# Mattdl/CLsurvey

Measured on AMD Instinct MI355X. Metric: images/sec (train+importance pass), EWC small_VGG9 Tiny-ImageNet task batch, higher is better.
Workload: dtype f32 (bf16x6 split operands on the conv fwd/bwd-data matrix products, fp32 accumulate); 1 GPU; EWC small_VGG9_cl_128_128, Tiny-ImageNet shapes (3x64x64, 20 classes), batch 200: train step + Fisher step (BASELINE configs[1]); batch=200, parallelism=1 GPU

## Files before the change

clsurvey_amd/_lib.py:

```python
import ctypes as C
import os

_HERE = os.path.dirname(os.path.abspath(__file__))
LIB_PATH = os.path.join(_HERE, "libclhip.so")

_p = C.c_void_p
_i = C.c_int
_f = C.c_float
_z = C.c_size_t
_l = C.c_long


class HatParam(C.Structure):
    _fields_ = [("theta", _p), ("grad", _p), ("buf", _p), ("mask_back", _p), ("n", _z), ("is_emb", _i), ("reserved", _i)]


class HatGateJob(C.Structure):
    _fields_ = [("emb_row", _p), ("gate", _p), ("mask_pre", _p), ("n", _i), ("reserved", _i)]


class HatLayer(C.Structure):
    _fields_ = [("w", _p), ("gate_in", _p), ("out", _p), ("K", _z), ("C", _z), ("R", _z)]


# ... 92 lines not shown
    "clhip_axpy": (_i, [_p, _p, _z, _f, _i, _p]),
    "clhip_gem_gram_ws": (_z, [_i]),
    "clhip_gem_gram": (_i, [_p, _z, C.POINTER(_i), _i, _z, _p, _p, _z, _p]),
    "clhip_gem_project": (_i, [_p, _z, C.POINTER(_i), C.POINTER(_f), _i, _p, _p, _z, _p]),
    "clhip_gem_qp": (_i, [_p, _i, C.c_double, C.c_double, _p, _p, _p]),
    "clhip_gem_project_dev": (_i, [_p, _z, C.POINTER(_i), _p, _p, _i, _p, _p, _z, _p]),
    "clhip_net_create": (_i, [C.POINTER(LayerDesc), _i, _i, _i, _i, _i, C.POINTER(_p)]),
    "clhip_net_set_dropout": (_i, [_p, _i, _p, _l]),
    "clhip_net_set_bn": (_i, [_p, _i, _p, _p, _f, _f]),
    "clhip_net_set_training": (_i, [_p, _i]),
    "clhip_net_probe": (_i, [_p, _i]),
    "clhip_net_probe_read": (_i, [_p, C.POINTER(_f), C.POINTER(_i)]),
    "clhip_net_layer_input": (_i, [_p, _i, _p, _p]),
    "clhip_net_layer_pool_idx": (_i, [_p, _i, _p, _p]),
    "clhip_net_layer_paths": (_i, [_p, _i]),
    "clhip_net_probe_kind": (_i, [_p, _i, _i]),
    "clhip_net_set_input_grad": (_i, [_p, _i, _p]),
    "clhip_sigmoid_fwd": (_i, [_p, _p, _z, _p]),
    "clhip_sigmoid_bwd": (_i, [_p, _p, _p, _z, _p]),
    "clhip_mse_mean": (_i, [_p, _p, _z, _f, _p, _p, _p]),
    "clhip_adadelta_step": (_i, [_p, _p, _p, _p, _z, _f, _f, _f, _f, _p]),
    "clhip_bn_ws": (_z, [_i]),
    "clhip_bn_fwd": (_i, [_p, _p, _p, _p, _p, _p, _p, _p, _i, _i, _i, _i, _f, _f, _i, _p, _z, _p]),
    "clhip_bn_bwd": (_i, [_p, _p, _p, _p, _p, _p, _p, _p, _p, _i, _i, _i, _i, _i, _p, _z, _p]),
    "clhip_net_destroy": (None, [_p]),
    "clhip_net_workspace_bytes": (_z, [_p]),
    "clhip_net_num_classes": (_i, [_p]),
    "clhip_net_forward": (_i, [_p, _p, _p, _i, _p, _p, _p]),
    "clhip_net_backward": (_i, [_p, _p, _p, _p, _i, _p, _p, _p]),
    "clhip_net_loss_step": (_i, [_p, _p, _p, _p, _p, _i, _i, _p, _p, _p, _p, _p]),
# ... 40 lines not shown
```

clsurvey_amd/csrc/bswgrad.hip:

```cpp
#include "common.hpp"
#include <cstdlib>

namespace {

typedef __bf16 bw_bf16x8 __attribute__((ext_vector_type(8)));
typedef __bf16 bw_bf16x2 __attribute__((ext_vector_type(2)));
typedef float bw_f32x2 __attribute__((ext_vector_type(2)));


__device__ __forceinline__ unsigned bw_pk(float lo, float hi) {
    bw_f32x2 v = {lo, hi};
    return __builtin_bit_cast(unsigned, __builtin_convertvector(v, bw_bf16x2));
}
__device__ __forceinline__ void bw_split2(float a, float b, unsigned& p0, unsigned& p1, unsigned& p2) {
    p0 = bw_pk(a, b);
    float ra = a - __uint_as_float(p0 << 16), rb = b - __uint_as_float(p0 & 0xffff0000u);
    p1 = bw_pk(ra, rb);
    ra -= __uint_as_float(p1 << 16);
    rb -= __uint_as_float(p1 & 0xffff0000u);
    p2 = bw_pk(ra, rb);
}

struct BwA { clhip_u32x4 p[3]; };
struct BwB { unsigned p[3][5]; };

__device__ __forceinline__ bw_bf16x8 bw_op(unsigned a, unsigned b, unsigned c, unsigned d) {
    return __builtin_bit_cast(bw_bf16x8, clhip_u32x4{a, b, c, d});
}
template <int S>
__device__ __forceinline__ bw_bf16x8 bw_tap(const BwB& b, int i) {
    if constexpr (S == 0) return bw_op(b.p[i][0], b.p[i][1], b.p[i][2], b.p[i][3]);
    else if constexpr (S == 2) return bw_op(b.p[i][1], b.p[i][2], b.p[i][3], b.p[i][4]);
    else return bw_op(__builtin_amdgcn_alignbit(b.p[i][1], b.p[i][0], 16), __builtin_amdgcn_alignbit(b.p[i][2], b.p[i][1], 16),
                      __builtin_amdgcn_alignbit(b.p[i][3], b.p[i][2], 16), __builtin_amdgcn_alignbit(b.p[i][4], b.p[i][3], 16));
}

#if BW_ABL & 1
__device__ __forceinline__ floatx16 bw_fake_mfma(bw_bf16x8 a, bw_bf16x8 b, floatx16 c) {
    c[0] += __builtin_bit_cast(clhip_u32x4, a).x == 0x12345678u ? 1.f : 0.f;
    c[1] += __builtin_bit_cast(clhip_u32x4, b).y == 0x12345678u ? 1.f : 0.f;
    return c;
}
#define BW_MFMA(a, b, c) bw_fake_mfma(a, b, c)
#else
#define BW_MFMA(a, b, c) __builtin_amdgcn_mfma_f32_32x32x16_bf16(a, b, c, 0, 0, 0)
#endif

struct BwRawX { float4 lo, hi; float l, r; };
struct BwRawD { float4 lo, hi; unsigned codes; };

#ifndef BW_ABL
#define BW_ABL 0
#endif
#ifndef BW_SCHED
#define BW_SCHED 1
#endif

template <bool UNPOOL>
__global__ __launch_bounds__(256, 1) void bs_wgrad_kernel(const float* __restrict__ x, const float* __restrict__ dy,
                                                          const uint8_t* __restrict__ idx, float* __restrict__ part, int N, int C, int K,
                                                          int H, int W, int splits, long long rows_total, size_t slab_stride) {
    const int lane = threadIdx.x & 63, wave = threadIdx.x >> 6;
    const int col = lane & 31, half = lane >> 5;
    const int split = blockIdx.x % splits, bt = blockIdx.x / splits;
    const int c_tiles = C >> 6;
    const int ct = bt % c_tiles, kt = bt / c_tiles;
    const int k0 = kt * 64 + (wave & 1) * 32, c0 = ct * 64 + (wave >> 1) * 32;
    const int strips = W >> 4;
// ... 240 lines not shown
```

clsurvey_amd/csrc/common.hpp:

```cpp
#pragma once
#include <hip/hip_runtime.h>
#include <stdint.h>
#include <stddef.h>
#include "../../include/clhip.h"

#define CLHIP_LAUNCH_CHECK()                          \
    do {                                              \
        hipError_t e__ = hipGetLastError();           \
        if (e__ != hipSuccess) return (int)e__;       \
    } while (0)

static inline hipStream_t as_stream(void* s) { return reinterpret_cast<hipStream_t>(s); }

static inline bool aligned16(const void* p) { return (reinterpret_cast<uintptr_t>(p) & 15u) == 0; }

static inline int ew_grid(size_t work_items, int block) {
    size_t g = (work_items + block - 1) / block;
    if (g < 1) g = 1;
    if (g > 2048) g = 2048;
    return (int)g;
}

static __device__ __attribute__((aligned(16))) float clhip_zero16[4] = {0.f, 0.f, 0.f, 0.f};

// ... 71 lines not shown
int clhip_internal_fc_bwd_combo(const clhip_gemm_args* g, int gemm_blocks, const clhip_fc_chain* d, float* grads, const float* x,
                                int N, const float* acts, const float* dlogits, const float* dz, hipStream_t s);

int clhip_internal_fc_tail_ok(const clhip_fc_chain* d);
int clhip_internal_fc_tail(const clhip_fc_chain* d, const float* params, float* acts, int N, const int64_t* labels,
                           int reduction, int col_off, int ncols, float* dlogits, float* fcdz, float* loss_out, double* stats,
                           void* row_scratch, unsigned* counter, int do_loss, int do_bwd, const float* h1_slabs, int live,
                           hipStream_t s);
int clhip_internal_fc_fwd_partial(const float* x, const float* w, int M, int I, int O, void* ws, size_t ws_bytes, int* live,
                                  hipStream_t s);

#define CLHIP_WGRAD_JOBS_MAX 32
struct clhip_wgrad_job { const float* part; float* dw; float* db; int K, C, splits; int taps; };
int clhip_internal_conv3x3_wgrad_partial(const float* x, const float* dy, const uint8_t* unpool_idx, float* dw, float* db, int N,
                                         int C, int K, int H, int W, void* ws, size_t ws_bytes, void* stream, clhip_wgrad_job* job);
int clhip_internal_wgrad_reduce_multi(const clhip_wgrad_job* jobs, int n, hipStream_t s);

bool clhip_internal_convkk_ok(int N, int Cin, int Cout, int H, int W, int R, int S, int stride, int pad);
int clhip_internal_convkk(int mode, const float* in, const float* w, const float* bias, const float* mask_src, float* out, int N,
                          int Cin, int Cout, int H, int W, int relu, hipStream_t s);

struct clhip_wino_wt { const float* w; float* U; int Ko, Ci, mode, pad; };
int clhip_internal_wino_weights(const clhip_wino_wt* jobs, int n, hipStream_t s);
int clhip_internal_weight_images(const clhip_wino_wt* wino_jobs, int n_wino, const clhip_wino_wt* bs_jobs, int n_bs, hipStream_t s);
int clhip_internal_wino_conv_u(int mode, const float* in, const float* U, const float* bias, const float* mask_src, float* out,
                               uint8_t* pool_idx, int unpool, int N, int Cin, int Cout, int H, int W, int relu, hipStream_t s);
bool clhip_internal_wino_ok(int Cin, int Cout, int H, int W);
size_t clhip_internal_wino_ws(int Cin, int Cout);
bool clhip_internal_bs_ok(int Cin, int Cout, int H, int W);
bool clhip_internal_bs_preferred(int Cin, int Cout, int H, int W);
// ... 32 lines not shown
```

clsurvey_amd/csrc/conv3x3_wgrad.hip:

```cpp
#include <cstdlib>
#include "common.hpp"

namespace {

constexpr int KT = 64, CT = 64;

#ifdef CLHIP_TRACE
__device__ unsigned long long* g_wtrace = nullptr;
#define TR_NOW() __builtin_amdgcn_s_memtime()
#endif

template <int TW, int TH>
struct WGeo {
    static constexpr int BP = TW * TH;
    static constexpr int TWP = TW + 2;
    static constexpr int PLANE = (TH + 2) * TWP;
    static constexpr int PLANEP = PLANE | 1;
    static constexpr int LDP = BP + 1;
    static_assert(BP == 64, "stage is 64 pixels");
};

__device__ __forceinline__ void decode_stage(int st, int tiles_w, int tiles_h, int TW, int TH,
                                             int& n, int& h0, int& w0) {
    int tw_i = st % tiles_w;
// ... 519 lines not shown
    }
}

#ifndef CLHIP_U3
#define CLHIP_U3 1
#endif
#ifndef CLHIP_U3_BSUM_MFMA
#define CLHIP_U3_BSUM_MFMA 0
#endif
#ifndef CLHIP_U3_LDSDY
#define CLHIP_U3_LDSDY 1
#endif
constexpr int U3_DYROW = 20, U3_DY = 32 * U3_DYROW;
constexpr int U3_TWP = 35, U3_PLANE = 3 * U3_TWP, U3_HALO = 3 * U3_PLANE + 5;

__global__ __launch_bounds__(256) void conv3x3_wgrad_c3_unpool_kernel(
    const float* __restrict__ x, const float* __restrict__ dyp, float* __restrict__ part,
    int N, int C, int K, int H, int W, int tiles_w, int tiles_h, int total_stages, int splits, size_t slab_stride,
    const uint8_t* __restrict__ pool_idx) {
    __shared__ float halo[4 * 2 * U3_HALO];
    __shared__ float red[2 * 16 * 64 + 64];
#if CLHIP_U3_LDSDY
    __shared__ __attribute__((aligned(16))) float dyl[4 * 2 * U3_DY];
#endif
#if CLHIP_U3_BSUM_MFMA
    __shared__ float ones_s[64];
    ones_s[threadIdx.x & 63] = 1.f;
    __syncthreads();
#endif
    const int tid = threadIdx.x, lane = tid & 63, wave = tid >> 6;
    const int wk = wave & 1, wh = wave >> 1;
    const int li = lane & 31, kk = lane >> 5;
    const int split = blockIdx.x % splits;
    const int kt = blockIdx.x / splits;
    const int k0 = kt * KT;
    const int per = total_stages / splits, extra = total_stages % splits;
    const int st_begin = split * per + min(split, extra);
    const int st_end = st_begin + per + (split < extra ? 1 : 0);

    floatx16 acc;
#pragma unroll
    for (int r = 0; r < 16; ++r) acc[r] = 0.f;
    double bsum = 0.0;

    const int ncol = C * 9;
    int col_off = 0;
    if (li < ncol) {
        const int cc = li / 9, rs = li - cc * 9;
        col_off = cc * U3_PLANE + (rs / 3) * U3_TWP + (rs % 3);
// ... 138 lines not shown
                if (kr < K) slab[((size_t)rs * K + kr) * C + cc] = acc[r] + red[(wk * 16 + r) * 64 + lane];
            }
        }
#if CLHIP_U3_BSUM_MFMA
        if (li == ncol) {
#pragma unroll
            for (int r = 0; r < 16; ++r) {
                const int kr = k0 + wk * 32 + mfma32_row(r, lane);
                if (kr < K) slab[(size_t)9 * K * C + kr] = acc[r] + red[(wk * 16 + r) * 64 + lane];
            }
        }
#else
        if (kk == 0 && kok) slab[(size_t)9 * K * C + k] = (float)(bsum + (double)red[2048 + wk * 32 + li]);
#endif
    }
}

constexpr int RED_EL = 64, RED_J = 16, RED_V = 4;
constexpr int RED_THREADS = RED_EL / RED_V * RED_J;

template <int EL, int J>
__device__ __forceinline__ void wgrad_reduce_block(const float* __restrict__ part, float* __restrict__ dw, float* __restrict__ db,
                                                   int K, int C, int splits, size_t e0, double (*partial)[EL], int T = 9) {
    const size_t kc = (size_t)K * C, nw = (size_t)T * kc, total = nw + K;
    const int v = threadIdx.x % (EL / RED_V), j = threadIdx.x / (EL / RED_V);
    const size_t e = e0 + (size_t)v * RED_V;
    const int q = (splits + J - 1) / J;
    const int s0 = j * q, s1 = min(splits, s0 + q);
    double s[RED_V] = {0.0, 0.0, 0.0, 0.0};
    if ((total & 3) == 0 && e + RED_V <= total) {
#pragma unroll 4
        for (int sp = s0; sp < s1; ++sp) {
            const float4 t = *reinterpret_cast<const float4*>(part + (size_t)sp * total + e);
            s[0] += (double)t.x; s[1] += (double)t.y; s[2] += (double)t.z; s[3] += (double)t.w;
        }
    } else {
        for (int sp = s0; sp < s1; ++sp)
#pragma unroll
            for (int t = 0; t < RED_V; ++t)
                if (e + t < total) s[t] += (double)part[(size_t)sp * total + e + t];
    }
#pragma unroll
    for (int t = 0; t < RED_V; ++t) partial[j][v * RED_V + t] = s[t];
    __syncthreads();
    if (threadIdx.x < EL) {
        const int el = threadIdx.x;
        const size_t ee = e0 + el;
        if (ee < total) {
            double t = 0.0;
#pragma unroll
            for (int jj = 0; jj < J; ++jj) t += partial[jj][el];
            if (ee < nw) {
                const size_t rs = ee / kc, rem = ee - rs * kc;
                dw[rem * T + rs] = (float)t;
            } else if (db) {
                db[ee - nw] = (float)t;
            }
        }
    }
}

template <int EL, int J>
__global__ __launch_bounds__(RED_THREADS) void wgrad_reduce_kernel(const float* __restrict__ part, float* __restrict__ dw,
                                                                   float* __restrict__ db, int K, int C, int splits) {
    __shared__ double partial[J][EL];
    wgrad_reduce_block<EL, J>(part, dw, db, K, C, splits, (size_t)blockIdx.x * EL, partial);
}

struct RedJobs {
    clhip_wgrad_job job[CLHIP_WGRAD_JOBS_MAX];
    unsigned first[CLHIP_WGRAD_JOBS_MAX + 1];
    int n;
};

template <int EL, int JL>
__global__ __launch_bounds__(RED_THREADS) void wgrad_reduce_multi_kernel(RedJobs jobs) {
    __shared__ double partial[JL][EL];
    int ji = 0;
    while (ji + 1 < jobs.n && blockIdx.x >= jobs.first[ji + 1]) ++ji;
    const clhip_wgrad_job J = jobs.job[ji];
    wgrad_reduce_block<EL, JL>(J.part, J.dw, J.db, J.K, J.C, J.splits, (size_t)(blockIdx.x - jobs.first[ji]) * EL, partial, J.taps ? J.taps : 9);
}

struct WPlan {
    int TW, TH, tiles_w, tiles_h, total_stages, splits, k_tiles, c_tiles, group, groups, ps;
    size_t slab, ws_floats;
};

WPlan make_plan(int N, int C, int K, int H, int W) {
    WPlan p;
    if (W > 16) { p.TW = 32; p.TH = 2; }
    else if (W > 8) { p.TW = 16; p.TH = 4; }
    else { p.TW = 8; p.TH = 8; }
    p.tiles_w = (W + p.TW - 1) / p.TW;
    p.tiles_h = (H + p.TH - 1) / p.TH;
    p.total_stages = p.tiles_w * p.tiles_h * N;
    const bool smallc = (C * 9 <= 32);
// ... 37 lines not shown

#ifdef CLHIP_TRACE
int clhip_debug_set_wgrad_trace(void* p) {
    unsigned long long* q = static_cast<unsigned long long*>(p);
    return (int)hipMemcpyToSymbol(HIP_SYMBOL(g_wtrace), &q, sizeof(q));
}
#endif

size_t clhip_conv3x3_bwd_weight_ws(int N, int C, int K, int H, int W) {
    if (N <= 0 || C <= 0 || K <= 0 || H <= 0 || W <= 0) return 0;
    return make_plan(N, C, K, H, W).ws_floats * sizeof(float);
}

static int bwd_weight_impl(const float* x, const float* dy, const uint8_t* unpool_idx, float* dw, float* db,
                           int N, int C, int K, int H, int W, void* ws, size_t ws_bytes, void* stream,
                           clhip_wgrad_job* defer = nullptr) {
    if (!x || !dy || !dw || !ws || N <= 0 || C <= 0 || K <= 0 || H <= 0 || W <= 0) return CLHIP_EINVAL;
    if (unpool_idx && ((H & 1) || (W & 1))) return CLHIP_ENOTSUP;
    WPlan p = make_plan(N, C, K, H, W);
    if (ws_bytes < p.ws_floats * sizeof(float)) return CLHIP_ENOSPC;
    hipStream_t s = as_stream(stream);
    float* part = static_cast<float*>(ws);
    const bool smallc = (C * 9 <= 32);
    unsigned grid = (unsigned)(p.k_tiles * p.c_tiles * p.splits);
#define WG_ARGS x, dy, part, N, C, K, H, W, p.tiles_w, p.tiles_h, p.total_stages, p.splits
    if (CLHIP_U3 && smallc && unpool_idx && p.TW == 32 && W % 32 == 0 && aligned16(dy) && aligned16(unpool_idx) &&
        (size_t)N * K * H * W < ((size_t)1 << 31) && (size_t)N * C * H * W < ((size_t)1 << 29)) {
        hipLaunchKernelGGL(conv3x3_wgrad_c3_unpool_kernel, dim3(grid), dim3(256), 0, s, WG_ARGS, p.slab, unpool_idx);
    } else if (smallc) {
        if (p.TW == 32) hipLaunchKernelGGL((conv3x3_wgrad_smallc_kernel<32, 2>), dim3(grid), dim3(256), 0, s, WG_ARGS, p.slab, unpool_idx);
        else if (p.TW == 16) hipLaunchKernelGGL((conv3x3_wgrad_smallc_kernel<16, 4>), dim3(grid), dim3(256), 0, s, WG_ARGS, p.slab, unpool_idx);
        else hipLaunchKernelGGL((conv3x3_wgrad_smallc_kernel<8, 8>), dim3(grid), dim3(256), 0, s, WG_ARGS, p.slab, unpool_idx);
    } else {
        const bool vec = (W % 4 == 0) && (W % p.TW == 0) && aligned16(x) && aligned16(dy);
        if (unpool_idx && (!vec || (reinterpret_cast<uintptr_t>(unpool_idx) & 1u))) return CLHIP_ENOTSUP;
#define WG_K(TW_, TH_, VEC_, PS_, UNP_) hipLaunchKernelGGL((conv3x3_wgrad_kernel<TW_, TH_, VEC_, PS_, UNP_>), dim3(grid), dim3(256), 0, s, \
                                                           WG_ARGS, p.c_tiles, p.slab, unpool_idx)
#define WG_LAUNCH1(TW_, TH_, PS_) do { if (unpool_idx) WG_K(TW_, TH_, true, PS_, true); else if (vec) WG_K(TW_, TH_, true, PS_, false); \
                                      else WG_K(TW_, TH_, false, PS_, false); } while (0)
#define WG_LAUNCH(TW_, TH_) do { if (p.ps) WG_LAUNCH1(TW_, TH_, true); else WG_LAUNCH1(TW_, TH_, false); } while (0)
        if (p.TW == 32) WG_LAUNCH(32, 2);
        else if (p.TW == 16) WG_LAUNCH(16, 4);
        else WG_LAUNCH(8, 8);
// ... 39 lines not shown
    const unsigned bx = (unsigned)((slab + RED_EL - 1) / RED_EL);
    hipLaunchKernelGGL((wgrad_reduce_kernel<RED_EL, RED_J>), dim3(bx), dim3(RED_THREADS), 0, as_stream(stream),
                            static_cast<const float*>(ws), dw, db, K, C, splits);
    CLHIP_LAUNCH_CHECK();
    return 0;
}

}

int clhip_internal_conv3x3_wgrad_partial(const float* x, const float* dy, const uint8_t* unpool_idx, float* dw, float* db, int N,
                                         int C, int K, int H, int W, void* ws, size_t ws_bytes, void* stream, clhip_wgrad_job* job) {
    if (!job) return CLHIP_EINVAL;
    return bwd_weight_impl(x, dy, unpool_idx, dw, db, N, C, K, H, W, ws, ws_bytes, stream, job);
}

int clhip_internal_wgrad_reduce_multi(const clhip_wgrad_job* jobs, int n, hipStream_t s) {
    if (n <= 0) return 0;
    if (!jobs || n > CLHIP_WGRAD_JOBS_MAX) return CLHIP_EINVAL;
    RedJobs r;
    r.n = n;
    r.first[0] = 0;
    for (int i = 0; i < n; ++i) {
        r.job[i] = jobs[i];
        const size_t total = (size_t)(jobs[i].taps ? jobs[i].taps : 9) * jobs[i].K * jobs[i].C + jobs[i].K;
        r.first[i + 1] = r.first[i] + (unsigned)((total + RED_EL - 1) / RED_EL);
    }
    for (int i = n; i < CLHIP_WGRAD_JOBS_MAX; ++i) { r.job[i] = clhip_wgrad_job{nullptr, nullptr, nullptr, 0, 0, 0, 0}; r.first[i + 1] = r.first[n]; }
    hipLaunchKernelGGL((wgrad_reduce_multi_kernel<RED_EL, RED_J>), dim3(r.first[n]), dim3(RED_THREADS), 0, s, r);
    CLHIP_LAUNCH_CHECK();
    return 0;
}
```

clsurvey_amd/csrc/engine.hip:

```cpp
#include <vector>
#include <cstdlib>
#include <new>
#include "common.hpp"

namespace {

struct LayerPlan {
    int type;
    int cin, cout, relu, pool;
    long w_off, b_off;
    int h, w;
    int ks, st, pd;
    int oh, ow;
    int pk, ps;
    int ph, pw;
    size_t in_elems, out_elems, pool_elems;
    size_t act_off;
    size_t pool_off;
    size_t idx_off;
    int bn;
    long bn_w_off, bn_b_off;
    size_t z_off;
    size_t stat_off;
    float* rmean; float* rvar; float bn_momentum, bn_eps;
// ... 40 lines not shown
    size_t off_wino;
    size_t off_s2d;
    int s2d_fresh_n;
    size_t total_bytes;
    size_t off_acts, off_idx, off_g0, off_g1, off_scratch, off_dlogits, off_loss, off_fcdz, off_wg;
    int training;
    int n_wg;
    int fc_first;
    bool fc_fused;
    clhip_fc_chain chain;
    int probe_layer;
    int probe_kind;
    unsigned probe_count;
    std::vector<hipEvent_t> probe_ev;
    bool fc_tail, no_combo;
    unsigned* tail_counter;
    size_t off_rows;
    bool overlap;
    int overlap_mode;
    hipStream_t side;
    std::vector<hipEvent_t> ev_dy, ev_wg;
    ~NetPlan() {
        for (hipEvent_t e : ev_dy) (void)hipEventDestroy(e);
        for (hipEvent_t e : ev_wg) (void)hipEventDestroy(e);
        if (side) (void)hipStreamDestroy(side);
        if (tail_counter) (void)hipFree(tail_counter);
        for (hipEvent_t e : probe_ev) (void)hipEventDestroy(e);
    }
};

// ... 230 lines not shown
            p->ev_dy.resize(n_layers); p->ev_wg.resize(n_layers);
            for (int i = 0; i < n_layers && p->overlap; ++i)
                if (hipEventCreateWithFlags(&p->ev_dy[i], hipEventDisableTiming) != hipSuccess ||
                    hipEventCreateWithFlags(&p->ev_wg[i], hipEventDisableTiming) != hipSuccess) p->overlap = false;
        } else {
            (void)hipGetLastError();
            p->side = nullptr;
        }
    }
    p->probe_layer = -1;
    p->probe_kind = 0;
    p->probe_count = 0;
    p->fc_tail = false;
    p->no_combo = false;
    p->tail_counter = nullptr;
    const char* tl = getenv("CLHIP_FC_TAIL");
    if (tl && tl[0] == '0') p->no_combo = true;
    if (p->fc_fused && !(tl && tl[0] == '0') && clhip_internal_fc_tail_ok(&p->chain) &&
        max_batch <= 1024) {
        if (hipMalloc(reinterpret_cast<void**>(&p->tail_counter), 256) == hipSuccess &&
            hipMemset(p->tail_counter, 0, 256) == hipSuccess) {
            p->fc_tail = true;
        } else {
            (void)hipGetLastError();
            if (p->tail_counter) { (void)hipFree(p->tail_counter); p->tail_counter = nullptr; }
        }
    }
    *out_handle = p;
    return 0;
}
// ... 19 lines not shown
    if (!p || layer <= 0 || layer >= (int)p->layers.size() || !ws_float_off || !in_elems) return CLHIP_EINVAL;
    const LayerPlan& P = p->layers[layer - 1];
    *ws_float_off = p->off_acts / sizeof(float) + ((P.type == 0 && P.pool) ? P.pool_off : P.act_off);
    *in_elems = p->layers[layer].in_elems;
    return 0;
}

int clhip_net_layer_pool_idx(void* handle, int layer, size_t* ws_byte_off, size_t* elems) {
    NetPlan* p = static_cast<NetPlan*>(handle);
    if (!p || layer < 0 || layer >= (int)p->layers.size() || !ws_byte_off || !elems) return CLHIP_EINVAL;
    const LayerPlan& L = p->layers[layer];
    if (L.type != 0 || !L.pool) return CLHIP_EINVAL;
    *ws_byte_off = p->off_idx + L.idx_off;
    *elems = L.pool_elems;
    return 0;
}

int clhip_net_layer_paths(void* handle, int layer) {
    NetPlan* p = static_cast<NetPlan*>(handle);
    if (!p || layer < 0 || layer >= (int)p->layers.size()) return CLHIP_EINVAL;
    const LayerPlan& L = p->layers[layer];
    const bool defer_capable = p->n_wg > 0 && !(p->overlap && p->overlap_mode == 1);
    return (L.wino_f ? 1 : 0) | (L.wino_d ? 2 : 0) | ((L.wino_w && defer_capable) ? 4 : 0) | ((L.bs_f || L.bs5_f) ? 8 : 0) |
           ((L.bs_d || L.bs5_d) ? 16 : 0) | ((L.bs_w && defer_capable) ? 32 : 0);
}

int clhip_net_set_input_grad(void* handle, int layer, const float* extra) {
    NetPlan* p = static_cast<NetPlan*>(handle);
    if (!p || layer <= 0 || layer >= (int)p->layers.size()) return CLHIP_EINVAL;
    p->layers[layer].extra_grad = extra;
// ... 246 lines not shown
    auto side_ok = [&](int layer) {
        if (ov) return true;
        const LayerPlan& Ls = p->layers[layer];
        return ov_small && Ls.type == 0 && Ls.wg3 && Ls.h * Ls.w <= 256;
    };
    hipEvent_t pending[2] = {nullptr, nullptr};
    hipEvent_t last_side = nullptr;
    int taken = -1;
    const bool defer = p->n_wg > 0 && !ov;
    auto pair_ok = [&](const LayerPlan& Lp, int layer) {
        return defer && layer > 0 && Lp.type == 0 && Lp.ks == 3 && Lp.st == 1 && Lp.pd == 1 && !Lp.bn && Lp.wino_w && Lp.wino_d &&
               !Lp.bs_d && !Lp.bs_w && Lp.wg_bytes && !Lp.drop && !Lp.extra_grad && !side_ok(layer);
    };
    clhip_wgrad_job jobs[CLHIP_WGRAD_JOBS_MAX];
    int n_jobs = 0;
    auto take = [&]() -> float* {
        const int bi = flip;
        flip ^= 1;
        if (pending[bi]) { (void)hipStreamWaitEvent(main_s, pending[bi], 0); pending[bi] = nullptr; }
        taken = bi;
        return g[bi];
    };
    auto on_side = [&](int layer, int dy_buf, auto&& launch) -> int {
        if (!side_ok(layer)) return launch(stream);
        hipError_t e = hipEventRecord(p->ev_dy[layer], main_s);
        if (e == hipSuccess) e = hipStreamWaitEvent(p->side, p->ev_dy[layer], 0);
        if (e != hipSuccess) return (int)e;
        const int r = launch((void*)p->side);
        if (r) return r;
        e = hipEventRecord(p->ev_wg[layer], p->side);
// ... 93 lines not shown
            if (!wdone) {
                probe_begin(2);
                rc = on_side(i, gin_buf, [&](void* st) {
                    if (defer && L.bs_w) {
                        const int r = clhip_internal_bs_wgrad_partial(xin, gin, idx + L.idx_off, grads + L.w_off, grads + L.b_off, N, L.cin,
                                                                      L.cout, L.h, L.w, base + p->off_wg + L.wg_off, L.wg_bytes, as_stream(st),
                                                                      &jobs[n_jobs]);
                        if (r != CLHIP_ENOTSUP && r != CLHIP_ENOSPC) return r;
                    }
                    if (defer && L.wino_w) {
                        const int r = clhip_internal_wino_wgrad_partial(xin, gin, idx + L.idx_off, grads + L.w_off, grads + L.b_off, N, L.cin,
                                                                        L.cout, L.h, L.w, base + p->off_wg + L.wg_off, L.wg_bytes,
                                                                        as_stream(st), &jobs[n_jobs]);
                        if (r != CLHIP_ENOTSUP && r != CLHIP_ENOSPC) return r;
                    }
                    if (defer)
                        return clhip_internal_conv3x3_wgrad_partial(xin, gin, idx + L.idx_off, grads + L.w_off, grads + L.b_off, N, L.cin,
                                                                    L.cout, L.h, L.w, base + p->off_wg + L.wg_off, L.wg_bytes, st,
                                                                    &jobs[n_jobs]);
                    return clhip_conv3x3_bwd_weight_unpool(xin, gin, idx + L.idx_off, grads + L.w_off, grads + L.b_off, N, L.cin, L.cout,
                                                           L.h, L.w, scratch, p->scratch_bytes, st);
                });
                if (rc == 0) { wdone = true; if (defer) ++n_jobs; probe_end(2); }
                else if (rc != CLHIP_ENOTSUP) return rc;
            }
            if (wdone && !ddone && i > 0 && !L.drop && !L.extra_grad) {
                if (!gout_d) { gout_d = take(); gout_d_buf = taken; }
                probe_begin(1);
                rc = L.wino_d ? plan_conv_u(L.bs_d, 1, gin, reinterpret_cast<const float*>(base + p->off_wino + L.wino_ud), nullptr,
                                                           xmask, gout_d, idx + L.idx_off, 1, N, L.cout, L.cin, L.h, L.w, 0, as_stream(stream))
// ... 184 lines not shown
```

clsurvey_amd/net.py:

```python
import ctypes as C
import weakref

import torch
import torch.nn as nn

from . import _lib
from ._lib import check, LayerDesc


def _pad4(n):
    return (n + 3) // 4 * 4


class ParamArena:
    _registry = weakref.WeakValueDictionary()

    @classmethod
    def find(cls, params):
        params = list(params)
        if not params:
            return None
        a = cls._registry.get(id(params[0]))
        if a is None or len(a.params) != len(params) or any(x is not y for x, y in zip(a.params, params)):
            return None
# ... 215 lines not shown
        lo = off.value * 4
        return self.ws[lo:lo + n * elems.value * 4].view(torch.float32).view(n, elems.value)

    def pool_idx(self, layer, n):
        off, elems = C.c_size_t(), C.c_size_t()
        check(_lib.lib().clhip_net_layer_pool_idx(self._h, int(layer), C.byref(off), C.byref(elems)), "clhip_net_layer_pool_idx")
        return self.ws[off.value:off.value + n * elems.value].view(n, elems.value)

    def layer_paths(self, layer):
        bits = _lib.lib().clhip_net_layer_paths(self._h, int(layer))
        if bits < 0:
            raise RuntimeError("clhip_net_layer_paths(%d)" % layer)
        return {"fwd": bool(bits & 1), "bwd_data": bool(bits & 2), "bwd_weight": bool(bits & 4),
                "bs_fwd": bool(bits & 8), "bs_bwd_data": bool(bits & 16), "bs_bwd_weight": bool(bits & 32)}

    def set_input_grad(self, layer, extra):
        if extra is not None and (not extra.is_cuda or extra.dtype != torch.float32 or not extra.is_contiguous()):
            raise RuntimeError("set_input_grad needs a contiguous fp32 HIP tensor")
        self._extra = extra
        check(_lib.lib().clhip_net_set_input_grad(self._h, int(layer), extra.data_ptr() if extra is not None else None),
              "clhip_net_set_input_grad")

    def _mode(self):
        if not self.bns:
            return
        training = bool(self.model.training)
        if training != self._training:
            check(_lib.lib().clhip_net_set_training(self._h, int(training)), "clhip_net_set_training")
            self._training = training
        if training:
# ... 83 lines not shown
```

include/clhip.h:

```cpp
#ifndef CLHIP_H
#define CLHIP_H

#include <stddef.h>
#include <stdint.h>

#ifdef __cplusplus
extern "C" {
#endif

#if defined(__GNUC__) || defined(__clang__)
#pragma GCC visibility push(default)
#define CLHIP_VISIBILITY_PUSHED 1
#endif

#define CLHIP_EINVAL (-1)
#define CLHIP_ENOSPC (-2)
#define CLHIP_ENOTSUP (-3)

int clhip_sigmoid_fwd(const float* x, float* y, size_t n, void* stream);
int clhip_sigmoid_bwd(const float* dy, const float* y, float* dx, size_t n, void* stream);
int clhip_mse_mean(const float* a, const float* b, size_t n, float grad_scale, float* da, float* loss_out, void* stream);
int clhip_adadelta_step(float* theta, const float* grad, float* square_avg, float* acc_delta, size_t n, float lr, float rho,
                        float eps, float weight_decay, void* stream);

// ... 167 lines not shown
    int bn;
    long bn_w_off, bn_b_off;
    int has_drop;
} clhip_layer_desc;

int clhip_net_create(const clhip_layer_desc* layers, int n_layers, int max_batch, int in_c, int in_h,
                     int in_w, void** out_handle);
int clhip_net_set_dropout(void* handle, int layer, const float* mask, long row_stride);
int clhip_net_set_bn(void* handle, int layer, float* running_mean, float* running_var, float momentum, float eps);
int clhip_net_set_training(void* handle, int training);
int clhip_net_probe(void* handle, int layer);
int clhip_net_probe_kind(void* handle, int layer, int kind);
int clhip_net_probe_read(void* handle, float* avg_us, int* count);
int clhip_net_layer_pool_idx(void* handle, int layer, size_t* ws_byte_off, size_t* elems_per_sample);
int clhip_net_layer_paths(void* handle, int layer);

int clhip_net_layer_input(void* handle, int layer, size_t* ws_float_off, size_t* in_elems);
int clhip_net_set_input_grad(void* handle, int layer, const float* extra);
void clhip_net_destroy(void* handle);
size_t clhip_net_workspace_bytes(void* handle);
int clhip_net_num_classes(void* handle);
int clhip_net_forward(void* handle, const float* params, const float* x, int N, void* ws,
                      float* logits_out, void* stream);
int clhip_net_backward(void* handle, const float* params, float* grads, const float* x, int N, void* ws,
                       const float* dlogits, void* stream);
int clhip_net_loss_step(void* handle, const float* params, float* grads, const float* x,
                        const int64_t* labels_i64, int N, int loss_kind, void* ws, float* loss_out,
                        double* stats, float* logits_out, void* stream);

int clhip_net_loss_step_slice(void* handle, const float* params, float* grads, const float* x,
// ... 34 lines not shown
```

Baseline: 280,100 images/s.

## Fold deferred wgrad split-reductions into the first-layer wgrad kernel launch

The split-K partial reductions deferred from the deeper conv layers now run inside the first-layer (3-channel, unpooled) wgrad kernel instead of in a separate reduce launch. Each block does rider reduction units either before or after its own work, chosen by a block-index bit (default position 16), or extra blocks are appended. This is meant to remove a kernel launch and to hide the reduction work under the memory-bound first-layer wgrad. The reduce kernel also gets a deeper unroll when the job count is small. Costs are larger LDS reuse and register pressure in the main kernel, and possible load imbalance between blocks.

```diff
diff --git a/clsurvey_amd/_lib.py b/clsurvey_amd/_lib.py
--- a/clsurvey_amd/_lib.py
+++ b/clsurvey_amd/_lib.py
@@ -130,6 +130,7 @@
     "clhip_net_layer_input": (_i, [_p, _i, _p, _p]),
     "clhip_net_layer_pool_idx": (_i, [_p, _i, _p, _p]),
     "clhip_net_layer_paths": (_i, [_p, _i]),
+    "clhip_net_last_ride": (_i, [_p]),
     "clhip_net_probe_kind": (_i, [_p, _i, _i]),
     "clhip_net_set_input_grad": (_i, [_p, _i, _p]),
     "clhip_sigmoid_fwd": (_i, [_p, _p, _z, _p]),
diff --git a/clsurvey_amd/csrc/bswgrad.hip b/clsurvey_amd/csrc/bswgrad.hip
--- a/clsurvey_amd/csrc/bswgrad.hip
+++ b/clsurvey_amd/csrc/bswgrad.hip
@@ -35,6 +35,9 @@
                       __builtin_amdgcn_alignbit(b.p[i][3], b.p[i][2], 16), __builtin_amdgcn_alignbit(b.p[i][4], b.p[i][3], 16));
 }
 
+#ifndef BW_ABL
+#define BW_ABL 0
+#endif
 #if BW_ABL & 1
 __device__ __forceinline__ floatx16 bw_fake_mfma(bw_bf16x8 a, bw_bf16x8 b, floatx16 c) {
     c[0] += __builtin_bit_cast(clhip_u32x4, a).x == 0x12345678u ? 1.f : 0.f;
@@ -49,9 +52,6 @@
 struct BwRawX { float4 lo, hi; float l, r; };
 struct BwRawD { float4 lo, hi; unsigned codes; };
 
-#ifndef BW_ABL
-#define BW_ABL 0
-#endif
 #ifndef BW_SCHED
 #define BW_SCHED 1
 #endif
diff --git a/clsurvey_amd/csrc/common.hpp b/clsurvey_amd/csrc/common.hpp
--- a/clsurvey_amd/csrc/common.hpp
+++ b/clsurvey_amd/csrc/common.hpp
@@ -109,6 +109,9 @@
 struct clhip_wgrad_job { const float* part; float* dw; float* db; int K, C, splits; int taps; };
 int clhip_internal_conv3x3_wgrad_partial(const float* x, const float* dy, const uint8_t* unpool_idx, float* dw, float* db, int N,
                                          int C, int K, int H, int W, void* ws, size_t ws_bytes, void* stream, clhip_wgrad_job* job);
+int clhip_internal_conv3x3_wgrad_partial_ride(const float* x, const float* dy, const uint8_t* unpool_idx, float* dw, float* db, int N,
+                                              int C, int K, int H, int W, void* ws, size_t ws_bytes, void* stream, clhip_wgrad_job* job,
+                                              const clhip_wgrad_job* riders, int n_riders, int* rode);
 int clhip_internal_wgrad_reduce_multi(const clhip_wgrad_job* jobs, int n, hipStream_t s);
 
 bool clhip_internal_convkk_ok(int N, int Cin, int Cout, int H, int W, int R, int S, int stride, int pad);
diff --git a/clsurvey_amd/csrc/conv3x3_wgrad.hip b/clsurvey_amd/csrc/conv3x3_wgrad.hip
--- a/clsurvey_amd/csrc/conv3x3_wgrad.hip
+++ b/clsurvey_amd/csrc/conv3x3_wgrad.hip
@@ -4,6 +4,77 @@
 namespace {
 
 constexpr int KT = 64, CT = 64;
+
+constexpr int RED_EL = 64, RED_J = 16, RED_V = 4;
+constexpr int RED_THREADS = RED_EL / RED_V * RED_J;
+
+template <int EL, int J, int UN = 4>
+__device__ __forceinline__ void wgrad_reduce_block(const float* __restrict__ part, float* __restrict__ dw, float* __restrict__ db,
+                                                   int K, int C, int splits, size_t e0, double (*partial)[EL], int T = 9) {
+    const size_t kc = (size_t)K * C, nw = (size_t)T * kc, total = nw + K;
+    const int v = threadIdx.x % (EL / RED_V), j = threadIdx.x / (EL / RED_V);
+    const size_t e = e0 + (size_t)v * RED_V;
+    const int q = (splits + J - 1) / J;
+    const int s0 = j * q, s1 = min(splits, s0 + q);
+    double s[RED_V] = {0.0, 0.0, 0.0, 0.0};
+    if ((total & 3) == 0 && e + RED_V <= total) {
+#pragma unroll UN
+        for (int sp = s0; sp < s1; ++sp) {
+            const float4 t = *reinterpret_cast<const float4*>(part + (size_t)sp * total + e);
+            s[0] += (double)t.x; s[1] += (double)t.y; s[2] += (double)t.z; s[3] += (double)t.w;
+        }
+    } else {
+        for (int sp = s0; sp < s1; ++sp)
+#pragma unroll
+            for (int t = 0; t < RED_V; ++t)
+                if (e + t < total) s[t] += (double)part[(size_t)sp * total + e + t];
+    }
+#pragma unroll
+    for (int t = 0; t < RED_V; ++t) partial[j][v * RED_V + t] = s[t];
+    __syncthreads();
+    if (threadIdx.x < EL) {
+        const int el = threadIdx.x;
+        const size_t ee = e0 + el;
+        if (ee < total) {
+            double t = 0.0;
+#pragma unroll
+            for (int jj = 0; jj < J; ++jj) t += partial[jj][el];
+            if (ee < nw) {
+                const size_t rs = ee / kc, rem = ee - rs * kc;
+                dw[rem * T + rs] = (float)t;
+            } else if (db) {
+                db[ee - nw] = (float)t;
+            }
+        }
+    }
+}
+
+struct RedJobs {
+    clhip_wgrad_job job[CLHIP_WGRAD_JOBS_MAX];
+    unsigned first[CLHIP_WGRAD_JOBS_MAX + 1];
+    int n;
+};
+
+RedJobs red_jobs(const clhip_wgrad_job* jobs, int n) {
+    RedJobs r;
+    r.n = n;
+    r.first[0] = 0;
+    for (int i = 0; i < n; ++i) {
+        r.job[i] = jobs[i];
+        const size_t total = (size_t)(jobs[i].taps ? jobs[i].taps : 9) * jobs[i].K * jobs[i].C + jobs[i].K;
+        r.first[i + 1] = r.first[i] + (unsigned)((total + RED_EL - 1) / RED_EL);
+    }
+    for (int i = n; i < CLHIP_WGRAD_JOBS_MAX; ++i) { r.job[i] = clhip_wgrad_job{nullptr, nullptr, nullptr, 0, 0, 0, 0}; r.first[i + 1] = r.first[n]; }
+    return r;
+}
+
+template <int EL, int JL, int UN = 4>
+__device__ __forceinline__ void wgrad_reduce_jobs_block(const RedJobs& jobs, unsigned block, double (*partial)[EL]) {
+    int ji = 0;
+    while (ji + 1 < jobs.n && block >= jobs.first[ji + 1]) ++ji;
+    const clhip_wgrad_job J = jobs.job[ji];
+    wgrad_reduce_block<EL, JL, UN>(J.part, J.dw, J.db, J.K, J.C, J.splits, (size_t)(block - jobs.first[ji]) * EL, partial, J.taps ? J.taps : 9);
+}
 
 #ifdef CLHIP_TRACE
 __device__ unsigned long long* g_wtrace = nullptr;
@@ -557,12 +628,44 @@
 constexpr int U3_DYROW = 20, U3_DY = 32 * U3_DYROW;
 constexpr int U3_TWP = 35, U3_PLANE = 3 * U3_TWP, U3_HALO = 3 * U3_PLANE + 5;
 
+__device__ __forceinline__ bool ride_map(unsigned b, unsigned main_blocks, unsigned riders, int ride_pos, unsigned& idx) {
+    if (ride_pos == 1) { idx = b < riders ? b : b - riders; return b < riders; }
+    if (ride_pos == 2) { idx = b < main_blocks ? b : b - main_blocks; return b >= main_blocks; }
+    const unsigned long long g = (unsigned long long)main_blocks + riders;
+    const unsigned before = (unsigned)((unsigned long long)b * main_blocks / g);
+    const bool is_main = (unsigned)((unsigned long long)(b + 1) * main_blocks / g) > before;
+    idx = is_main ? before : b - before;
+    return !is_main;
+}
+
+constexpr int RIDE_POS_DEFAULT = 8 + 8;
+
+template <bool RIDE>
 __global__ __launch_bounds__(256) void conv3x3_wgrad_c3_unpool_kernel(
     const float* __restrict__ x, const float* __restrict__ dyp, float* __restrict__ part,
     int N, int C, int K, int H, int W, int tiles_w, int tiles_h, int total_stages, int splits, size_t slab_stride,
-    const uint8_t* __restrict__ pool_idx) {
+    const uint8_t* __restrict__ pool_idx, RedJobs riders, unsigned main_blocks, int ride_pos) {
     __shared__ float halo[4 * 2 * U3_HALO];
-    __shared__ float red[2 * 16 * 64 + 64];
+    __shared__ __attribute__((aligned(16))) float red[2 * 16 * 64 + 64];
+    unsigned bid = blockIdx.x;
+    static_assert(sizeof(red) >= sizeof(double) * RED_J * RED_EL && RED_THREADS == 256, "rider work borrows `red` and the block shape");
+    [[maybe_unused]] auto ride_units = [&]() {
+        for (unsigned u = blockIdx.x; u < riders.first[riders.n]; u += main_blocks) {
+            wgrad_reduce_jobs_block<RED_EL, RED_J>(riders, u, reinterpret_cast<double (*)[RED_EL]>(red));
+            __syncthreads();
+        }
+    };
+    [[maybe_unused]] const bool ride_early = ride_pos >= 8 && ((blockIdx.x >> (ride_pos - 8)) & 1u);
+    if (RIDE) {
+        if (ride_pos < 8) {
+            if (ride_map(blockIdx.x, main_blocks, riders.first[riders.n], ride_pos, bid)) {
+                wgrad_reduce_jobs_block<RED_EL, RED_J>(riders, bid, reinterpret_cast<double (*)[RED_EL]>(red));
+                return;
+            }
+        } else if (ride_early) {
+            ride_units();
+        }
+    }
 #if CLHIP_U3_LDSDY
     __shared__ __attribute__((aligned(16))) float dyl[4 * 2 * U3_DY];
 #endif
@@ -574,8 +677,8 @@
     const int tid = threadIdx.x, lane = tid & 63, wave = tid >> 6;
     const int wk = wave & 1, wh = wave >> 1;
     const int li = lane & 31, kk = lane >> 5;
-    const int split = blockIdx.x % splits;
-    const int kt = blockIdx.x / splits;
+    const int split = bid % splits;
+    const int kt = bid / splits;
     const int k0 = kt * KT;
     const int per = total_stages / splits, extra = total_stages % splits;
     const int st_begin = split * per + min(split, extra);
@@ -744,49 +847,9 @@
         if (kk == 0 && kok) slab[(size_t)9 * K * C + k] = (float)(bsum + (double)red[2048 + wk * 32 + li]);
 #endif
     }
-}
-
-constexpr int RED_EL = 64, RED_J = 16, RED_V = 4;
-constexpr int RED_THREADS = RED_EL / RED_V * RED_J;
-
-template <int EL, int J>
-__device__ __forceinline__ void wgrad_reduce_block(const float* __restrict__ part, float* __restrict__ dw, float* __restrict__ db,
-                                                   int K, int C, int splits, size_t e0, double (*partial)[EL], int T = 9) {
-    const size_t kc = (size_t)K * C, nw = (size_t)T * kc, total = nw + K;
-    const int v = threadIdx.x % (EL / RED_V), j = threadIdx.x / (EL / RED_V);
-    const size_t e = e0 + (size_t)v * RED_V;
-    const int q = (splits + J - 1) / J;
-    const int s0 = j * q, s1 = min(splits, s0 + q);
-    double s[RED_V] = {0.0, 0.0, 0.0, 0.0};
-    if ((total & 3) == 0 && e + RED_V <= total) {
-#pragma unroll 4
-        for (int sp = s0; sp < s1; ++sp) {
-            const float4 t = *reinterpret_cast<const float4*>(part + (size_t)sp * total + e);
-            s[0] += (double)t.x; s[1] += (double)t.y; s[2] += (double)t.z; s[3] += (double)t.w;
-        }
-    } else {
-        for (int sp = s0; sp < s1; ++sp)
-#pragma unroll
-            for (int t = 0; t < RED_V; ++t)
-                if (e + t < total) s[t] += (double)part[(size_t)sp * total + e + t];
-    }
-#pragma unroll
-    for (int t = 0; t < RED_V; ++t) partial[j][v * RED_V + t] = s[t];
-    __syncthreads();
-    if (threadIdx.x < EL) {
-        const int el = threadIdx.x;
-        const size_t ee = e0 + el;
-        if (ee < total) {
-            double t = 0.0;
-#pragma unroll
-            for (int jj = 0; jj < J; ++jj) t += partial[jj][el];
-            if (ee < nw) {
-                const size_t rs = ee / kc, rem = ee - rs * kc;
-                dw[rem * T + rs] = (float)t;
-            } else if (db) {
-                db[ee - nw] = (float)t;
-            }
-        }
+    if (RIDE && ride_pos >= 8 && !ride_early) {
+        __syncthreads();
+        ride_units();
     }
 }
 
@@ -797,20 +860,12 @@
     wgrad_reduce_block<EL, J>(part, dw, db, K, C, splits, (size_t)blockIdx.x * EL, partial);
 }
 
-struct RedJobs {
-    clhip_wgrad_job job[CLHIP_WGRAD_JOBS_MAX];
-    unsigned first[CLHIP_WGRAD_JOBS_MAX + 1];
-    int n;
-};
-
-template <int EL, int JL>
+template <int EL, int JL, int UN>
 __global__ __launch_bounds__(RED_THREADS) void wgrad_reduce_multi_kernel(RedJobs jobs) {
     __shared__ double partial[JL][EL];
-    int ji = 0;
-    while (ji + 1 < jobs.n && blockIdx.x >= jobs.first[ji + 1]) ++ji;
-    const clhip_wgrad_job J = jobs.job[ji];
-    wgrad_reduce_block<EL, JL>(J.part, J.dw, J.db, J.K, J.C, J.splits, (size_t)(blockIdx.x - jobs.first[ji]) * EL, partial, J.taps ? J.taps : 9);
-}
+    wgrad_reduce_jobs_block<EL, JL, UN>(jobs, blockIdx.x, partial);
+}
+constexpr int RED_SMALL_BLOCKS = 256, RED_UN_SMALL = 16;
 
 struct WPlan {
     int TW, TH, tiles_w, tiles_h, total_stages, splits, k_tiles, c_tiles, group, groups, ps;
@@ -878,7 +933,8 @@
 
 static int bwd_weight_impl(const float* x, const float* dy, const uint8_t* unpool_idx, float* dw, float* db,
                            int N, int C, int K, int H, int W, void* ws, size_t ws_bytes, void* stream,
-                           clhip_wgrad_job* defer = nullptr) {
+                           clhip_wgrad_job* defer = nullptr, const clhip_wgrad_job* riders = nullptr, int n_riders = 0,
+                           int* rode = nullptr) {
     if (!x || !dy || !dw || !ws || N <= 0 || C <= 0 || K <= 0 || H <= 0 || W <= 0) return CLHIP_EINVAL;
     if (unpool_idx && ((H & 1) || (W & 1))) return CLHIP_ENOTSUP;
     WPlan p = make_plan(N, C, K, H, W);
@@ -890,7 +946,17 @@
 #define WG_ARGS x, dy, part, N, C, K, H, W, p.tiles_w, p.tiles_h, p.total_stages, p.splits
     if (CLHIP_U3 && smallc && unpool_idx && p.TW == 32 && W % 32 == 0 && aligned16(dy) && aligned16(unpool_idx) &&
         (size_t)N * K * H * W < ((size_t)1 << 31) && (size_t)N * C * H * W < ((size_t)1 << 29)) {
-        hipLaunchKernelGGL(conv3x3_wgrad_c3_unpool_kernel, dim3(grid), dim3(256), 0, s, WG_ARGS, p.slab, unpool_idx);
+        if (riders && n_riders > 0 && n_riders <= CLHIP_WGRAD_JOBS_MAX) {
+            static const int pos_env = [] { const char* e = getenv("CLHIP_WG_RIDE_POS"); return e && e[0] ? atoi(e) : 0; }();
+            const int pos = (pos_env >= 1 && pos_env <= 3) || (pos_env >= 8 && pos_env < 40) ? pos_env : RIDE_POS_DEFAULT;
+            const RedJobs r = red_jobs(riders, n_riders);
+            hipLaunchKernelGGL(conv3x3_wgrad_c3_unpool_kernel<true>, dim3(grid + (pos < 8 ? r.first[n_riders] : 0u)), dim3(256), 0, s,
+                               WG_ARGS, p.slab, unpool_idx, r, grid, pos);
+            if (rode) *rode = n_riders;
+        } else {
+            hipLaunchKernelGGL(conv3x3_wgrad_c3_unpool_kernel<false>, dim3(grid), dim3(256), 0, s, WG_ARGS, p.slab, unpool_idx, RedJobs{},
+                               grid, 0);
+        }
     } else if (smallc) {
         if (p.TW == 32) hipLaunchKernelGGL((conv3x3_wgrad_smallc_kernel<32, 2>), dim3(grid), dim3(256), 0, s, WG_ARGS, p.slab, unpool_idx);
         else if (p.TW == 16) hipLaunchKernelGGL((conv3x3_wgrad_smallc_kernel<16, 4>), dim3(grid), dim3(256), 0, s, WG_ARGS, p.slab, unpool_idx);
@@ -960,19 +1026,23 @@
     return bwd_weight_impl(x, dy, unpool_idx, dw, db, N, C, K, H, W, ws, ws_bytes, stream, job);
 }
 
+int clhip_internal_conv3x3_wgrad_partial_ride(const float* x, const float* dy, const uint8_t* unpool_idx, float* dw, float* db, int N,
+                                              int C, int K, int H, int W, void* ws, size_t ws_bytes, void* stream, clhip_wgrad_job* job,
+                                              const clhip_wgrad_job* riders, int n_riders, int* rode) {
+    if (!job || !rode) return CLHIP_EINVAL;
+    *rode = 0;
+    return bwd_weight_impl(x, dy, unpool_idx, dw, db, N, C, K, H, W, ws, ws_bytes, stream, job, riders, n_riders, rode);
+}
+
 int clhip_internal_wgrad_reduce_multi(const clhip_wgrad_job* jobs, int n, hipStream_t s) {
     if (n <= 0) return 0;
     if (!jobs || n > CLHIP_WGRAD_JOBS_MAX) return CLHIP_EINVAL;
-    RedJobs r;
-    r.n = n;
-    r.first[0] = 0;
-    for (int i = 0; i < n; ++i) {
-        r.job[i] = jobs[i];
-        const size_t total = (size_t)(jobs[i].taps ? jobs[i].taps : 9) * jobs[i].K * jobs[i].C + jobs[i].K;
-        r.first[i + 1] = r.first[i] + (unsigned)((total + RED_EL - 1) / RED_EL);
-    }
-    for (int i = n; i < CLHIP_WGRAD_JOBS_MAX; ++i) { r.job[i] = clhip_wgrad_job{nullptr, nullptr, nullptr, 0, 0, 0, 0}; r.first[i + 1] = r.first[n]; }
-    hipLaunchKernelGGL((wgrad_reduce_multi_kernel<RED_EL, RED_J>), dim3(r.first[n]), dim3(RED_THREADS), 0, s, r);
+    const RedJobs r = red_jobs(jobs, n);
+    static const bool deep = [] { const char* e = getenv("CLHIP_TAIL_RIDE"); return !(e && e[0] == '0'); }();
+    if (deep && r.first[n] <= RED_SMALL_BLOCKS)
+        hipLaunchKernelGGL((wgrad_reduce_multi_kernel<RED_EL, RED_J, RED_UN_SMALL>), dim3(r.first[n]), dim3(RED_THREADS), 0, s, r);
+    else
+        hipLaunchKernelGGL((wgrad_reduce_multi_kernel<RED_EL, RED_J, 4>), dim3(r.first[n]), dim3(RED_THREADS), 0, s, r);
     CLHIP_LAUNCH_CHECK();
     return 0;
 }
diff --git a/clsurvey_amd/csrc/engine.hip b/clsurvey_amd/csrc/engine.hip
--- a/clsurvey_amd/csrc/engine.hip
+++ b/clsurvey_amd/csrc/engine.hip
@@ -78,6 +78,8 @@
     unsigned probe_count;
     std::vector<hipEvent_t> probe_ev;
     bool fc_tail, no_combo;
+    bool tail_ride;
+    int last_ride;
     unsigned* tail_counter;
     size_t off_rows;
     bool overlap;
@@ -338,6 +340,9 @@
     p->fc_tail = false;
     p->no_combo = false;
     p->tail_counter = nullptr;
+    const char* tr = getenv("CLHIP_TAIL_RIDE");
+    p->tail_ride = !(tr && tr[0] == '0');
+    p->last_ride = 0;
     const char* tl = getenv("CLHIP_FC_TAIL");
     if (tl && tl[0] == '0') p->no_combo = true;
     if (p->fc_fused && !(tl && tl[0] == '0') && clhip_internal_fc_tail_ok(&p->chain) &&
@@ -387,6 +392,11 @@
     *ws_byte_off = p->off_idx + L.idx_off;
     *elems = L.pool_elems;
     return 0;
+}
+
+int clhip_net_last_ride(void* handle) {
+    NetPlan* p = static_cast<NetPlan*>(handle);
+    return p ? p->last_ride : CLHIP_EINVAL;
 }
 
 int clhip_net_layer_paths(void* handle, int layer) {
@@ -663,6 +673,13 @@
     };
     clhip_wgrad_job jobs[CLHIP_WGRAD_JOBS_MAX];
     int n_jobs = 0;
+    bool ride = p->tail_ride && defer && !p->overlap;
+    for (const LayerPlan& Lr : p->layers) ride = ride && !Lr.bn && !Lr.drop && !Lr.extra_grad;
+    {
+        const LayerPlan& L0 = p->layers[0];
+        ride = ride && L0.type == 0 && L0.wg3 && L0.cin * 9 <= 32 && L0.pool && L0.pk == 2 && L0.ps == 2 && !L0.bs_w && !L0.wino_w;
+    }
+    p->last_ride = 0;
     auto take = [&]() -> float* {
         const int bi = flip;
         flip ^= 1;
@@ -786,6 +803,14 @@
                                                                         as_stream(st), &jobs[n_jobs]);
                         if (r != CLHIP_ENOTSUP && r != CLHIP_ENOSPC) return r;
                     }
+                    if (defer && ride && i == 0 && n_jobs > 0) {
+                        int rode = 0;
+                        const int r = clhip_internal_conv3x3_wgrad_partial_ride(xin, gin, idx + L.idx_off, grads + L.w_off, grads + L.b_off,
+                                                                                N, L.cin, L.cout, L.h, L.w, base + p->off_wg + L.wg_off,
+                                                                                L.wg_bytes, st, &jobs[n_jobs], jobs, n_jobs, &rode);
+                        if (r == 0 && rode) { p->last_ride = rode; jobs[0] = jobs[n_jobs]; n_jobs = 0; }
+                        return r;
+                    }
                     if (defer)
                         return clhip_internal_conv3x3_wgrad_partial(xin, gin, idx + L.idx_off, grads + L.w_off, grads + L.b_off, N, L.cin,
                                                                     L.cout, L.h, L.w, base + p->off_wg + L.wg_off, L.wg_bytes, st,
diff --git a/clsurvey_amd/net.py b/clsurvey_amd/net.py
--- a/clsurvey_amd/net.py
+++ b/clsurvey_amd/net.py
@@ -253,6 +253,12 @@
         return {"fwd": bool(bits & 1), "bwd_data": bool(bits & 2), "bwd_weight": bool(bits & 4),
                 "bs_fwd": bool(bits & 8), "bs_bwd_data": bool(bits & 16), "bs_bwd_weight": bool(bits & 32)}
 
+    def last_ride(self):
+        n = _lib.lib().clhip_net_last_ride(self._h)
+        if n < 0:
+            raise RuntimeError("clhip_net_last_ride")
+        return n
+
     def set_input_grad(self, layer, extra):
         if extra is not None and (not extra.is_cuda or extra.dtype != torch.float32 or not extra.is_contiguous()):
             raise RuntimeError("set_input_grad needs a contiguous fp32 HIP tensor")
diff --git a/include/clhip.h b/include/clhip.h
--- a/include/clhip.h
+++ b/include/clhip.h
@@ -205,6 +205,7 @@
 int clhip_net_probe_read(void* handle, float* avg_us, int* count);
 int clhip_net_layer_pool_idx(void* handle, int layer, size_t* ws_byte_off, size_t* elems_per_sample);
 int clhip_net_layer_paths(void* handle, int layer);
+int clhip_net_last_ride(void* handle);
 
 int clhip_net_layer_input(void* handle, int layer, size_t* ws_float_off, size_t* in_elems);
 int clhip_net_set_input_grad(void* handle, int layer, const float* extra);
```

New measurement: 281,400 images/s, median of 6. Within noise of the previous version (+0.4%).
